# bramtoula/multi_robot_SLAM_separators

Hardware: AMD Instinct MI355X
Metric: candidate keyframe-pair verifications/sec (NetVLAD NN + ORB match + RANSAC) @1/2/4/8 GPU (higher is better)
Workload: dtype u8+f16+f32+f64

## Files before the change

### multi_robot_slam_separators_amd/csrc/k_match.hip

```cpp
#include "sf_internal.hpp"
#include <type_traits>

namespace {

__device__ __forceinline__ uint32_t bcnt_acc(uint32_t x, uint32_t acc) {
  uint32_t r;
  asm("v_bcnt_u32_b32 %0, %1, %2" : "=v"(r) : "v"(x), "v"(acc));
  return r;
}

template <int W, int NQ>
__device__ __forceinline__ void knn2_scan(const uint32_t* __restrict__ dF, int Kf, const uint32_t (&q)[NQ][W],
                                          uint32_t (&k1)[NQ], uint32_t (&k2)[NQ]) {
#pragma unroll 4
  for (int f = 0; f < Kf; ++f) {
    const uint32_t* r = dF + (size_t)f * W;
    uint32_t x[W];
#pragma unroll
    for (int c = 0; c < W; ++c) x[c] = r[c];
#pragma unroll
    for (int j = 0; j < NQ; ++j) {
      uint32_t d = 0;
#pragma unroll
      for (int c = 0; c < W; ++c) d = bcnt_acc(x[c] ^ q[j][c], d);
      const uint32_t key = (d << 16) | (uint32_t)f;
      k2[j] = min(max(key, k1[j]), k2[j]);
      k1[j] = min(k1[j], key);
    }
  }
}

template <int W>
__device__ __forceinline__ void knn2_scan_l2(const uint32_t* __restrict__ dF, int Kf, const uint32_t (&q)[W], float& d1,
                                             float& d2, int& i1) {
#pragma unroll 1
  for (int f = 0; f < Kf; ++f) {
    const uint32_t* r = dF + (size_t)f * W;
    float s = 0.f;
#pragma unroll
    for (int c = 0; c < W; ++c) {
      const float d = __uint_as_float(q[c]) - __uint_as_float(r[c]);
      s = s + d * d;
    }
    if (s < d1) { d2 = d1; d1 = s; i1 = f; }
    else if (s < d2) { d2 = s; }
  }
}

template <int W>
__device__ __forceinline__ void knn2_scan_l2_halves(const uint32_t* __restrict__ dF, int Kf,
                                                    const uint32_t* __restrict__ qrow, float& d1, float& d2, int& i1) {
  static_assert(W == 128, "two halves of 64 dimensions");
  constexpr int H = 64, FB = 16;
#pragma unroll 1
  for (int f0 = 0; f0 < Kf; f0 += FB) {
    float s[FB];
#pragma unroll
    for (int j = 0; j < FB; ++j) s[j] = 0.f;
#pragma unroll 1
    for (int half = 0; half < 2; ++half) {
      uint32_t q[H];
      {
        const uint4* p = reinterpret_cast<const uint4*>(qrow + half * H);
#pragma unroll
        for (int c = 0; c < H / 4; ++c) {
          const uint4 v = p[c];
          q[4 * c] = v.x; q[4 * c + 1] = v.y; q[4 * c + 2] = v.z; q[4 * c + 3] = v.w;
        }
      }
#pragma unroll
      for (int j = 0; j < FB; ++j) {
        if (f0 + j < Kf) {
          const uint32_t* r = dF + (size_t)(f0 + j) * W + half * H;
          float a = s[j];
#pragma unroll
          for (int c = 0; c < H; ++c) {
            const float d = __uint_as_float(q[c]) - __uint_as_float(r[c]);
            a = a + d * d;
          }
          s[j] = a;
        }
      }
    }
#pragma unroll
    for (int j = 0; j < FB; ++j) {
      if (f0 + j < Kf) {
        if (s[j] < d1) { d2 = d1; d1 = s[j]; i1 = f0 + j; }
        else if (s[j] < d2) { d2 = s[j]; }
      }
    }
  }
}

template <int W>
__device__ __forceinline__ void load_desc(const uint32_t* __restrict__ base, int row, bool valid, uint32_t (&q)[W]) {
  const uint4* p = reinterpret_cast<const uint4*>(base + (size_t)(valid ? row : 0) * W);
#pragma unroll
  for (int c = 0; c < W / 4; ++c) {
    uint4 v = p[c];
    q[4 * c + 0] = v.x; q[4 * c + 1] = v.y; q[4 * c + 2] = v.z; q[4 * c + 3] = v.w;
  }
}

template <int W, int NQ, int NT, bool L2 = false>
__global__ void __launch_bounds__(NT)
k_match_global(StoreView st, const int32_t* __restrict__ pair_from, const int32_t* __restrict__ pair_to,
               float nndr, int min_inliers, int est, uint32_t* __restrict__ corr, CorrHeader* __restrict__ hdr,
               PassState* __restrict__ pass, int32_t* __restrict__ list, int32_t* __restrict__ counter) {
  extern __shared__ __attribute__((aligned(16))) int smem[];
  constexpr int NW = NT / 64;
  const int pair = blockIdx.x;
  const int tid = threadIdx.x;
  const int lane = tid & 63, wave = tid >> 6;
  const int kcap = st.kcap;
  const int sF = pair_from[pair], sT = pair_to[pair];
  if ((unsigned)sF >= (unsigned)st.n_slots || (unsigned)sT >= (unsigned)st.n_slots) {
    if (tid == 0) {
      CorrHeader h = {0, 0, 0, 0};
      hdr[pair] = h;
      PassState ps;
#pragma unroll
      for (int i = 0; i < 12; ++i) ps.T[i] = 0.f;
      ps.var = 1.0; ps.var_ang = 1.0; ps.is_null = 1; ps.inliers = 0; ps.matches = 0; ps.pad = 0;
      pass[pair] = ps;
    }
    return;
  }
  const int4 mF = st.meta[sF], mT = st.meta[sT];
  const int Kf = mF.x, Kt = mT.x;
  const uint32_t* dF = st.desc + (size_t)sF * kcap * W;
  const uint32_t* dT = st.desc + (size_t)sT * kcap * W;

  int* cnt = smem;
  int* owner = smem + kcap;
  int* misc = smem + 2 * kcap;

  for (int i = tid; i < Kf; i += NT) cnt[i] = 0;
  if (tid < 16) misc[tid] = 0;
  __syncthreads();

  int rejected = 0;
  if constexpr (L2) {
    static_assert(!L2 || NQ == 1, "one resident float row per lane");
    if (Kf > 0) {
      for (int base = 0; base < Kt; base += NT) {
        const int t = base + tid;
        float d1 = __int_as_float(0x7F800000), d2 = __int_as_float(0x7F800000);
        int i1 = -1;
        if constexpr (W > 64) {
          if (Kt - base - (tid & ~63) > 0)
            knn2_scan_l2_halves<W>(dF, Kf, dT + (size_t)(t < Kt ? t : 0) * W, d1, d2, i1);
        } else {
          uint32_t q[W];
          load_desc<W>(dT, t, t < Kt, q);
          if (Kt - base - (tid & ~63) > 0)
            knn2_scan_l2<W>(dF, Kf, q, d1, d2, i1);
        }
        if (t < Kt) {
          const bool acc = (Kf >= 2) && i1 >= 0 && !(d1 > nndr * d2);
          if (acc) {
            atomicAdd(&cnt[i1], 1);
            owner[i1] = t;
          } else {
            ++rejected;
          }
        }
      }
    }
  } else
  if (Kf > 0) {
    for (int base = 0; base < Kt; base += NQ * NT) {
      uint32_t q[NQ][W], k1[NQ], k2[NQ];
#pragma unroll
      for (int j = 0; j < NQ; ++j) {
        const int t = base + j * NT + tid;
        load_desc<W>(dT, t, t < Kt, q[j]);
        k1[j] = 0xFFFFFFFFu;
        k2[j] = 0xFFFFFFFFu;
      }
      const int wave_rows = Kt - base - (tid & ~63);
      const int groups = wave_rows <= 0 ? 0 : min(NQ, (wave_rows + NT - 1) / NT);
      if (groups == NQ) {
        knn2_scan<W, NQ>(dF, Kf, q, k1, k2);
      } else if (groups > 0) {
#pragma unroll
        for (int j = 0; j < NQ; ++j) {
          if (j < groups) {
            uint32_t qq[1][W], a1[1] = {0xFFFFFFFFu}, a2[1] = {0xFFFFFFFFu};
#pragma unroll
            for (int c = 0; c < W; ++c) qq[0][c] = q[j][c];
            knn2_scan<W, 1>(dF, Kf, qq, a1, a2);
            k1[j] = a1[0];
            k2[j] = a2[0];
          }
        }
      }
#pragma unroll
      for (int j = 0; j < NQ; ++j) {
        const int t = base + j * NT + tid;
        if (t < Kt) {
          const bool acc = (Kf >= 2) && !((float)(k1[j] >> 16) > nndr * (float)(k2[j] >> 16));
          if (acc) {
            const int f = (int)(k1[j] & 0xFFFFu);
            atomicAdd(&cnt[f], 1);
            owner[f] = t;
          } else {
            ++rejected;
          }
        }
      }
    }
  }
  for (int off = 32; off >= 1; off >>= 1) rejected += __shfl_xor(rejected, off);
  if (lane == 0 && rejected) atomicAdd(&misc[0], rejected);
  __syncthreads();

  uint32_t* out = corr + (size_t)pair * kcap;
  int running = 0;
  for (int base = 0; base < Kf; base += NT) {
    const int f = base + tid;
    const bool flag = (f < Kf) && (cnt[f] == 1);
    const unsigned long long bal = __ballot(flag);
    const int before = __popcll(bal & ((1ull << lane) - 1ull));
    if (lane == 0) misc[4 + wave] = __popcll(bal);
    __syncthreads();
    int woff = 0, total = 0;
#pragma unroll
    for (int w = 0; w < NW; ++w) {
      int c = misc[4 + w];
      if (w < wave) woff += c;
      total += c;
    }
    if (flag) out[running + woff + before] = (uint32_t)f | ((uint32_t)owner[f] << 16);
    running += total;
    __syncthreads();
  }
  const int n_corr = running;

  const int unique_to = (Kf > 0 && Kt > 0) ? misc[0] + n_corr : 0;
  const int words_from = (Kf > 0 && mF.y > 0) ? Kf : 0;
  const int words_to = (mT.y > 0) ? unique_to : 0;
  const bool motion = est == 0 ? (unique_to > 0 && words_from >= min_inliers && words_to >= min_inliers)
                    : est == 1 ? (unique_to > 0 && words_from >= min_inliers && unique_to >= min_inliers)
                               : (est == 3 && unique_to > 0 && ((words_from >= min_inliers && unique_to >= min_inliers) ||
                                                                (words_to >= min_inliers && Kf >= min_inliers)));
  const bool survivor = est == 3 ? (motion && n_corr > 0) : (motion && n_corr >= min_inliers && n_corr >= (est == 0 ? 3 : 4));
  if (motion && !survivor) {
    const float* xF = st.xyz + (size_t)sF * kcap * 3;
    const float* xT = st.xyz + (size_t)sT * kcap * 3;
    for (int i = tid; i < n_corr; i += NT) {
      uint32_t c = out[i];
      const float* a = xF + 3 * (c & 0xFFFFu);
      const float* b = xT + 3 * (c >> 16);
      bool ok = isfinite(a[0]) && isfinite(a[1]) && isfinite(a[2]);
      if (est == 0)
        ok = ok && isfinite(b[0]) && isfinite(b[1]) && isfinite(b[2]) && (a[0] != 0.f || a[1] != 0.f || a[2] != 0.f) &&
             (b[0] != 0.f || b[1] != 0.f || b[2] != 0.f);
      if (ok) atomicAdd(&misc[2], 1);
    }
    __syncthreads();
  }
  if (tid == 0) {
    CorrHeader h;
    h.n_corr = n_corr;
    h.words_from = words_from;
    h.words_to = words_to;
    h.words_to_2d = unique_to;
    hdr[pair] = h;
    PassState ps;
#pragma unroll
    for (int i = 0; i < 12; ++i) ps.T[i] = 0.f;
    ps.var = 1.0; ps.var_ang = 1.0;
    ps.is_null = 1;
    ps.inliers = 0;
    ps.matches = (motion && !survivor) ? misc[2] : 0;
    ps.pad = 0;
    pass[pair] = ps;
    if (survivor) {
      int pos = atomicAdd(counter, 1);
      list[pos] = pair;
    }
  }
}

__device__ __forceinline__ uint32_t min_u16(uint32_t a, uint32_t b) {
  uint32_t r;
  asm("v_min_u16 %0, %1, %2" : "=v"(r) : "v"(a), "v"(b));
  return r;
}
__device__ __forceinline__ uint32_t max_u16(uint32_t a, uint32_t b) {
  uint32_t r;
  asm("v_max_u16 %0, %1, %2" : "=v"(r) : "v"(a), "v"(b));
  return r;
}

constexpr int MATCH_CH = 16;

template <int W, int NQ>
__device__ __forceinline__ void knn2_step_lds(const uint32_t* fromD, int f, const uint32_t (&q)[NQ][W],
                                              uint32_t (&d1)[NQ], uint32_t (&d2)[NQ]) {
  const uint4* r = reinterpret_cast<const uint4*>(fromD + (size_t)f * W);
  uint32_t x[W];
#pragma unroll
  for (int c = 0; c < W / 4; ++c) {
    const uint4 v = r[c];
    x[4 * c] = v.x; x[4 * c + 1] = v.y; x[4 * c + 2] = v.z; x[4 * c + 3] = v.w;
  }
#pragma unroll
  for (int j = 0; j < NQ; ++j) {
    uint32_t d = 0;
#pragma unroll
    for (int c = 0; c < W; ++c) d = bcnt_acc(x[c] ^ q[j][c], d);
    d2[j] = min_u16(d2[j], max_u16(d, d1[j]));
    d1[j] = min_u16(d1[j], d);
  }
}

template <int W, int NQ>
__device__ __forceinline__ void knn2_scan_lds(const uint32_t* fromD, int Kf, const uint32_t (&q)[NQ][W],
                                              uint32_t (&d1)[NQ], uint32_t (&d2)[NQ], uint32_t (&chunk)[NQ]) {
  int c0 = 0;
  for (; c0 + MATCH_CH <= Kf; c0 += MATCH_CH) {
    uint32_t prev[NQ];
#pragma unroll
    for (int j = 0; j < NQ; ++j) prev[j] = d1[j];
#pragma unroll 4
    for (int u = 0; u < MATCH_CH; ++u) knn2_step_lds<W, NQ>(fromD, c0 + u, q, d1, d2);
#pragma unroll
    for (int j = 0; j < NQ; ++j) chunk[j] = ((d1[j] & 0xFFFFu) != (prev[j] & 0xFFFFu)) ? (uint32_t)c0 : chunk[j];
  }
  if (c0 < Kf) {
    uint32_t prev[NQ];
#pragma unroll
    for (int j = 0; j < NQ; ++j) prev[j] = d1[j];
    for (int f = c0; f < Kf; ++f) knn2_step_lds<W, NQ>(fromD, f, q, d1, d2);
#pragma unroll
    for (int j = 0; j < NQ; ++j) chunk[j] = ((d1[j] & 0xFFFFu) != (prev[j] & 0xFFFFu)) ? (uint32_t)c0 : chunk[j];
  }
}

typedef int mf_v8i __attribute__((ext_vector_type(8)));
typedef float mf_v16f __attribute__((ext_vector_type(16)));
constexpr float MF_FR = 1.f / 2048.f;
constexpr int MF_MAX_ROWS = 2048;

__device__ __forceinline__ mf_v8i fp4_spread_from(uint32_t x, uint32_t m88, uint32_t c22) {
  mf_v8i o = {0, 0, 0, 0, 0, 0, 0, 0};
  o[0] = (int)((x & m88) | c22);
  o[1] = (int)(x & 0x44444444u);
  o[2] = (int)(x & 0x22222222u);
  o[3] = (int)(x & 0x11111111u);
  return o;
}
__device__ __forceinline__ mf_v8i fp4_spread_to(uint32_t y, uint32_t m88, uint32_t c22) {
  mf_v8i o = {0, 0, 0, 0, 0, 0, 0, 0};
  const uint32_t n = ~y;
  o[0] = (int)((y & m88) | c22);
  o[1] = (int)(((n << 1) & m88) | c22);
  o[2] = (int)(((n << 2) & m88) | 0x44444444u);
  o[3] = (int)(((n << 3) & m88) | 0x66666666u);
  return o;
}

static inline size_t sf_match_lds_bytes(int kcap, int w) {
  const int behind = 2 * kcap + 16;
  return (size_t)(kcap * w + (behind > 32 * w ? behind : 32 * w)) * sizeof(int);
}

template <int KS>
__device__ __forceinline__ void load_raw(const uint32_t* p, uint32_t (&raw)[KS]) {
#pragma unroll
  for (int c = 0; c < KS / 4; ++c) {
    const uint4 v = reinterpret_cast<const uint4*>(p)[c];
    raw[4 * c] = v.x; raw[4 * c + 1] = v.y; raw[4 * c + 2] = v.z; raw[4 * c + 3] = v.w;
  }
}

__device__ __forceinline__ void top2_update16(const mf_v16f& v, float& b, float& s) {
  float t = __builtin_amdgcn_fmed3f(v[0], v[1], INFINITY);
  float x;
  asm("v_max3_f32 %[t], %[t], %[o2], %[o3]\n\t"
      "v_max3_f32 %[t], %[t], %[o4], %[o5]\n\t"
      "v_max3_f32 %[t], %[t], %[o6], %[o7]\n\t"
      "v_max3_f32 %[t], %[t], %[o8], %[o9]\n\t"
      "v_max3_f32 %[t], %[t], %[o10], %[o11]\n\t"
      "v_max3_f32 %[t], %[t], %[o12], %[o13]\n\t"
      "v_max_f32 %[t], %[t], %[o14]\n\t"
      "v_med3_f32 %[x], %[b], %[t], %[o15]\n\t"
      "v_max3_f32 %[b], %[b], %[t], %[o15]\n\t"
      "v_max_f32 %[s], %[s], %[x]"
      : [b] "+v"(b), [s] "+v"(s), [t] "+v"(t), [x] "=&v"(x)
      : [o2] "v"(v[2]), [o3] "v"(v[3]), [o4] "v"(v[4]), [o5] "v"(v[5]), [o6] "v"(v[6]), [o7] "v"(v[7]), [o8] "v"(v[8]),
        [o9] "v"(v[9]), [o10] "v"(v[10]), [o11] "v"(v[11]), [o12] "v"(v[12]), [o13] "v"(v[13]), [o14] "v"(v[14]),
        [o15] "v"(v[15]));
}

template <int W, int NTL, bool TAIL>
__device__ __forceinline__ void knn2_mfma_tile(const uint32_t* fromD, int Kf, int mt, int r, int h,
                                               const mf_v8i (&Bf)[NTL][W / 2], const float (&cin)[16],
                                               float (&b)[NTL], float (&s)[NTL], uint32_t m88, uint32_t c22,
                                               uint32_t (&raw)[W / 2], const uint32_t*& nxt) {
  constexpr int KS = W / 2;
  mf_v16f c0;
#pragma unroll
  for (int i = 0; i < 16; ++i) c0[i] = cin[i];
  if (TAIL) {
    const float lim = -(float)(Kf - mt * 32) * MF_FR;
#pragma unroll
    for (int i = 0; i < 16; ++i) c0[i] = c0[i] > lim ? c0[i] : -INFINITY;
  }
  mf_v8i Af[KS];
#pragma unroll
  for (int k = 0; k < KS; ++k) Af[k] = fp4_spread_from(raw[k], m88, c22);
  if (!TAIL) {
    nxt += 32 * W;
    load_raw<KS>(nxt, raw);
  }
#pragma unroll
  for (int j = 0; j < NTL; ++j) {
    b[j] += 32.f * MF_FR;
    s[j] += 32.f * MF_FR;
  }
#pragma unroll
  for (int j = 0; j < NTL; ++j) {
    mf_v16f acc = __builtin_amdgcn_mfma_scale_f32_32x32x64_f8f6f4(Af[0], Bf[j][0], c0, 4, 4, 0, 0, 0, 0);
#pragma unroll
    for (int k = 1; k < KS; ++k)
      acc = __builtin_amdgcn_mfma_scale_f32_32x32x64_f8f6f4(Af[k], Bf[j][k], acc, 4, 4, 0, 0, 0, 0);
    top2_update16(acc, b[j], s[j]);
  }
}

template <int W, int NTL>
struct MfB {
  mf_v8i Bf[NTL][W / 2];
  uint32_t psum;
};

template <int W, int NTL>
__device__ __forceinline__ void mf_load_b(const uint32_t* __restrict__ dT, int Kt, const int (&tile)[NTL], int lane,
                                          MfB<W, NTL>& B) {
  constexpr int KS = W / 2;
  const int r = lane & 31, h = lane >> 5;
  uint32_t m88, c22;
  asm volatile("v_mov_b32 %0, 0x88888888" : "=v"(m88));
  asm volatile("v_mov_b32 %0, 0x22222222" : "=v"(c22));
  uint32_t raw[NTL][KS];
#pragma unroll
  for (int j = 0; j < NTL; ++j) load_raw<KS>(dT + (size_t)min(tile[j] * 32 + r, Kt - 1) * W + KS * h, raw[j]);
  static_assert(NTL == 1 || 24 * W < 256, "a tile's popcount fits its byte");
  uint32_t pk = 0;
#pragma unroll
  for (int j = 0; j < NTL; ++j) {
    uint32_t p = 0;
#pragma unroll
    for (int k = 0; k < KS; ++k) {
      B.Bf[j][k] = fp4_spread_to(raw[j][k], m88, c22);
      p += __popc(raw[j][k] & 0x77777777u);
    }
    pk |= p << (8 * j);
  }
  B.psum = pk + __shfl_xor(pk, 32);
}

typedef int mf_v4i __attribute__((ext_vector_type(4)));

__device__ __forceinline__ void mf_pipe_half1(mf_v16f& acc, const mf_v4i& a0, const mf_v4i& a1, const mf_v4i& a2,
                                              const mf_v4i& a3, const mf_v4i& b0, const mf_v4i& b1, const mf_v16f& cin,
                                              const mf_v16f& old, float& b, float& s, float& t) {
  asm volatile(
      "s_nop 1\n\t"
      "v_mfma_f32_32x32x64_f8f6f4 %[acc], %[a0], %[b0], %[cin] cbsz:4 blgp:4\n\t"
      "v_add_f32 %[b], 0x3c800000, %[b]\n\t"
      "v_add_f32 %[s], 0x3c800000, %[s]\n\t"
      "s_nop 4\n\t"
      "v_max3_f32 %[t], %[o0], %[o1], %[o2]\n\t"
      "v_mfma_f32_32x32x64_f8f6f4 %[acc], %[a1], %[b1], %[acc] cbsz:4 blgp:4\n\t"
      "v_max3_f32 %[t], %[t], %[o3], %[o4]\n\t"
      "v_max3_f32 %[t], %[t], %[o5], %[o6]\n\t"
      "v_max3_f32 %[t], %[t], %[o7], %[o8]"
      : [acc] "=&v"(acc), [b] "+v"(b), [s] "+v"(s), [t] "=&v"(t)
      : [a0] "v"(a0), [a1] "v"(a1), "v"(a2), "v"(a3), [b0] "v"(b0), [b1] "v"(b1), [cin] "v"(cin), [o0] "v"(old[0]),
        [o1] "v"(old[1]), [o2] "v"(old[2]), [o3] "v"(old[3]), [o4] "v"(old[4]), [o5] "v"(old[5]), [o6] "v"(old[6]),
        [o7] "v"(old[7]), [o8] "v"(old[8]));
}
__device__ __forceinline__ void mf_pipe_half2(mf_v16f& acc, const mf_v4i& a2, const mf_v4i& a3, const mf_v4i& b2,
                                              const mf_v4i& b3, const mf_v16f& old, float& b, float& s, float& t) {
  float x;
  asm volatile(
      "v_mfma_f32_32x32x64_f8f6f4 %[acc], %[a2], %[b2], %[acc] cbsz:4 blgp:4\n\t"
      "v_max3_f32 %[t], %[t], %[o9], %[o10]\n\t"
      "v_max3_f32 %[t], %[t], %[o11], %[o12]\n\t"
      "v_max3_f32 %[t], %[t], %[o13], %[o14]\n\t"
      "v_mfma_f32_32x32x64_f8f6f4 %[acc], %[a3], %[b3], %[acc] cbsz:4 blgp:4\n\t"
      "v_med3_f32 %[x], %[b], %[t], %[o15]\n\t"
      "v_max3_f32 %[b], %[b], %[t], %[o15]\n\t"
      "v_max_f32 %[s], %[s], %[x]"
      : [acc] "+v"(acc), [b] "+v"(b), [s] "+v"(s), [t] "+v"(t), [x] "=&v"(x)
      : [a2] "v"(a2), [a3] "v"(a3), [b2] "v"(b2), [b3] "v"(b3), [o9] "v"(old[9]), [o10] "v"(old[10]), [o11] "v"(old[11]),
        [o12] "v"(old[12]), [o13] "v"(old[13]), [o14] "v"(old[14]), [o15] "v"(old[15]));
}
__device__ __forceinline__ void mf_pipe_drain(const mf_v16f& old, float& b, float& s) {
  float t, x;
  asm volatile(
      "s_nop 11\n\t"
      "v_add_f32 %[b], 0x3c800000, %[b]\n\t"
      "v_add_f32 %[s], 0x3c800000, %[s]\n\t"
      "v_max3_f32 %[t], %[o0], %[o1], %[o2]\n\t"
      "v_max3_f32 %[t], %[t], %[o3], %[o4]\n\t"
      "v_max3_f32 %[t], %[t], %[o5], %[o6]\n\t"
      "v_max3_f32 %[t], %[t], %[o7], %[o8]\n\t"
      "v_max3_f32 %[t], %[t], %[o9], %[o10]\n\t"
      "v_max3_f32 %[t], %[t], %[o11], %[o12]\n\t"
      "v_max3_f32 %[t], %[t], %[o13], %[o14]\n\t"
      "v_med3_f32 %[x], %[b], %[t], %[o15]\n\t"
      "v_max3_f32 %[b], %[b], %[t], %[o15]\n\t"
      "v_max_f32 %[s], %[s], %[x]"
      : [b] "+v"(b), [s] "+v"(s), [t] "=&v"(t), [x] "=&v"(x)
      : [o0] "v"(old[0]), [o1] "v"(old[1]), [o2] "v"(old[2]), [o3] "v"(old[3]), [o4] "v"(old[4]), [o5] "v"(old[5]),
        [o6] "v"(old[6]), [o7] "v"(old[7]), [o8] "v"(old[8]), [o9] "v"(old[9]), [o10] "v"(old[10]), [o11] "v"(old[11]),
        [o12] "v"(old[12]), [o13] "v"(old[13]), [o14] "v"(old[14]), [o15] "v"(old[15]));
}

template <int NTL>
__device__ __forceinline__ void mf_scan_tiles_pipe(const uint32_t* fromD, int n_full, int tail, const MfB<8, NTL>& B,
                                                   const float (&cin)[16], float (&b)[NTL], float (&s)[NTL],
                                                   uint32_t m88, uint32_t c22, uint32_t (&raw)[4],
                                                   const uint32_t*& nxt) {
  static_assert(NTL == 2 || NTL == 4, "tiles alternate between two accumulator tuples");
  mf_v4i B4[NTL][4];
#pragma unroll
  for (int j = 0; j < NTL; ++j) {
#pragma unroll
    for (int k = 0; k < 4; ++k) B4[j][k] = mf_v4i{B.Bf[j][k][0], B.Bf[j][k][1], B.Bf[j][k][2], B.Bf[j][k][3]};
  }
  mf_v16f c0, acc0, acc1;
#pragma unroll
  for (int i = 0; i < 16; ++i) { c0[i] = cin[i]; acc1[i] = -INFINITY; }
#pragma unroll 1
  for (int pass = 0; pass < 2; ++pass) {
    int n = n_full, step = 32 * 8;
    if (pass) {
      if (!tail) break;
      const float lim = -(float)tail * MF_FR;
#pragma unroll
      for (int i = 0; i < 16; ++i) c0[i] = c0[i] > lim ? c0[i] : -INFINITY;
      n = 1; step = 0;
    }
    for (int mt = 0; mt < n; ++mt) {
      mf_v4i A4[4];
#pragma unroll
      for (int k = 0; k < 4; ++k) {
        const mf_v8i a = fp4_spread_from(raw[k], m88, c22);
        A4[k] = mf_v4i{a[0], a[1], a[2], a[3]};
      }
      nxt += step;
      load_raw<4>(nxt, raw);
#pragma unroll
      for (int j = 0; j < NTL; j += 2) {
        constexpr int JP = NTL - 1;
        float t;
        const int jp = j == 0 ? JP : j - 1;
        mf_pipe_half1(acc0, A4[0], A4[1], A4[2], A4[3], B4[j][0], B4[j][1], c0, acc1, b[jp], s[jp], t);
        mf_pipe_half2(acc0, A4[2], A4[3], B4[j][2], B4[j][3], acc1, b[jp], s[jp], t);
        mf_pipe_half1(acc1, A4[0], A4[1], A4[2], A4[3], B4[j + 1][0], B4[j + 1][1], c0, acc0, b[j], s[j], t);
        mf_pipe_half2(acc1, A4[2], A4[3], B4[j + 1][2], B4[j + 1][3], acc0, b[j], s[j], t);
      }
    }
  }
  mf_pipe_drain(acc1, b[NTL - 1], s[NTL - 1]);
}

__device__ __forceinline__ float mf_max(float a, float b) {
  float r;
  asm("v_max_f32 %0, %1, %2" : "=v"(r) : "v"(a), "v"(b));
  return r;
}
__device__ __forceinline__ float mf_min(float a, float b) {
  float r;
  asm("v_min_f32 %0, %1, %2" : "=v"(r) : "v"(a), "v"(b));
  return r;
}
__device__ __forceinline__ float mf_max3(float a, float b, float c) {
  float r;
  asm("v_max3_f32 %0, %1, %2, %3" : "=v"(r) : "v"(a), "v"(b), "v"(c));
  return r;
}

constexpr int mf_passes(int ntl) { return ntl == 1 ? 1 : ntl / 2; }

template <int W, int NTL, bool PIPE = false>
__device__ __forceinline__ void mf_scan(const uint32_t* fromD, int Kf, const MfB<W, NTL>& B, int lane,
                                        uint32_t (&d1)[mf_passes(NTL)], uint32_t (&d2)[mf_passes(NTL)],
                                        int (&idx)[mf_passes(NTL)]) {
  constexpr int KS = W / 2;
  const int r = lane & 31, h = lane >> 5;
  uint32_t m88, c22;
  asm volatile("v_mov_b32 %0, 0x88888888" : "=v"(m88));
  asm volatile("v_mov_b32 %0, 0x22222222" : "=v"(c22));
  float cin[16], b[NTL], s[NTL];
  const float hoff = h ? 4.f * MF_FR : 0.f;
#pragma unroll
  for (int i = 0; i < 16; ++i) cin[i] = -(float)((i & 3) + 8 * (i >> 2)) * MF_FR - hoff;
#pragma unroll
  for (int j = 0; j < NTL; ++j) { b[j] = -INFINITY; s[j] = -INFINITY; }
  const int n_full = Kf >> 5;
  uint32_t raw[KS];
  load_raw<KS>(fromD + (size_t)min(r, Kf - 1) * W + KS * h, raw);
  const uint32_t* nxt = fromD + (size_t)r * W + KS * h;
  if constexpr (PIPE && W == 8 && (NTL == 2 || NTL == 4)) {
    mf_scan_tiles_pipe<NTL>(fromD, n_full, Kf & 31, B, cin, b, s, m88, c22, raw, nxt);
  } else {
    for (int mt = 0; mt < n_full; ++mt) knn2_mfma_tile<W, NTL, false>(fromD, Kf, mt, r, h, B.Bf, cin, b, s, m88, c22, raw, nxt);
    if (Kf & 31) knn2_mfma_tile<W, NTL, true>(fromD, Kf, n_full, r, h, B.Bf, cin, b, s, m88, c22, raw, nxt);
  }
  const float org = (float)(32 * (((Kf + 31) >> 5) - 1)) * MF_FR;
#pragma unroll
  for (int p = 0; p < mf_passes(NTL); ++p) {
    float mb, ms, ob, os;
    int ts;
    if constexpr (NTL == 1) {
      mb = b[0]; ms = s[0]; ts = 24 * W - 2 * (int)B.psum;
      ob = __shfl_xor(mb, 32); os = __shfl_xor(ms, 32);
    } else {
      const int j0 = 2 * p, j1 = 2 * p + 1;
      mb = h ? b[j1] : b[j0]; ms = h ? s[j1] : s[j0]; ts = 24 * W - 2 * (int)((B.psum >> (16 * p + 8 * h)) & 0xFFu);
      ob = __shfl_xor(h ? b[j0] : b[j1], 32); os = __shfl_xor(h ? s[j0] : s[j1], 32);
    }
    const float nb = mf_max(mb, ob) - org;
    const float ns = mf_max3(mf_min(mb, ob), ms, os) - org;
    const float dot1 = 2.f * ceilf(nb * 0.5f), dot2 = 2.f * ceilf(ns * 0.5f);
    idx[p] = (int)((dot1 - nb) * 2048.f);
    d1[p] = (uint32_t)((32 * W - ts - (int)dot1) >> 1);
    d2[p] = ns == -INFINITY ? 0xFFFFu : (uint32_t)((32 * W - ts - (int)dot2) >> 1);
  }
}

template <int W, int NTL, bool PIPE = false>
__device__ __forceinline__ void knn2_mfma(const uint32_t* fromD, int Kf, const uint32_t* __restrict__ dT, int Kt,
                                          const int (&tile)[NTL], int lane, uint32_t (&d1)[mf_passes(NTL)],
                                          uint32_t (&d2)[mf_passes(NTL)], int (&idx)[mf_passes(NTL)]) {
  asm volatile("" : "+v"(lane));
  MfB<W, NTL> B;
  mf_load_b<W, NTL>(dT, Kt, tile, lane, B);
  mf_scan<W, NTL, PIPE>(fromD, Kf, B, lane, d1, d2, idx);
}

template <int W>
__device__ __forceinline__ uint32_t mf_repair_d2(const uint32_t* fromD, int Kf, const uint32_t* __restrict__ q_row, int idx,
                                                 uint32_t d2) {
  if ((idx & 27) == 27) return d2;
  uint32_t q[W];
  load_raw<W>(q_row, q);
  const int base = (idx & ~31) + (idx & 4);
#pragma unroll 1
  for (int g = 0; g < 32; g += 8) {
#pragma unroll
    for (int k = 0; k < 4; ++k) {
      const int row = base + g + k;
      uint32_t x[W];
      load_raw<W>(fromD + (size_t)row * W, x);
      uint32_t d = 0;
#pragma unroll
      for (int c = 0; c < W; ++c) d = bcnt_acc(x[c] ^ q[c], d);
      const bool other = row < Kf && row != idx && (g + k) != 27;
      d2 = other ? min(d2, d) : d2;
    }
  }
  return d2;
}

template <int W, int NQ, int NT, int MF_NTL = 2, bool MF_PIPE = false>
__device__ __forceinline__ bool match_v2_body(const StoreView& st, int pair, int sF, int sT, float nndr, int min_inliers,
                                              int est, uint32_t* out, CorrHeader& hdr_out, PassState& pass_out,
                                              int32_t* __restrict__ list, int32_t* __restrict__ counter, int* smem,
                                              unsigned long long* trace_row = nullptr) {
  constexpr int NW = NT / 64;
  const int tid = threadIdx.x;
  const int lane = tid & 63, wave = __builtin_amdgcn_readfirstlane(tid >> 6);
  const int kcap = st.kcap;
  if ((unsigned)sF >= (unsigned)st.n_slots || (unsigned)sT >= (unsigned)st.n_slots) {
    if (tid == 0) {
      CorrHeader h = {0, 0, 0, 0};
      hdr_out = h;
      PassState ps;
#pragma unroll
      for (int i = 0; i < 12; ++i) ps.T[i] = 0.f;
      ps.var = 1.0; ps.var_ang = 1.0; ps.is_null = 1; ps.inliers = 0; ps.matches = 0; ps.pad = 0;
      pass_out = ps;
    }
    return false;
  }
  const int4 mF = st.meta[sF], mT = st.meta[sT];
  const int Kf = mF.x, Kt = mT.x;
  const uint32_t* dF = st.desc + (size_t)sF * kcap * W;
  const uint32_t* dT = st.desc + (size_t)sT * kcap * W;

  uint32_t* fromD = reinterpret_cast<uint32_t*>(smem);
  int* cnt = smem + kcap * W;
  int* owner = cnt + kcap;
  int* misc = owner + kcap;

  {
    const uint4* src = reinterpret_cast<const uint4*>(dF);
    uint4* dst = reinterpret_cast<uint4*>(fromD);
    for (int i = tid; i < Kf * (W / 4); i += NT) dst[i] = src[i];
  }
  for (int i = tid; i < Kf; i += NT) cnt[i] = 0;
  if (tid < 16) misc[tid] = 0;
  __syncthreads();
  SF_TRACE_ROW_MARK(trace_row, 32);

  int rejected = 0;
  if constexpr (NQ == 0) {
    if (Kf > 0) {
      constexpr int NTL = W == 8 ? MF_NTL : 1;
      const int n_nt = (Kt + 31) >> 5;
      auto group = [&](auto g, int t0) {
        constexpr int G = decltype(g)::value, NP = mf_passes(G);
        int tl[G], f[NP];
        uint32_t a1[NP], a2[NP];
#pragma unroll
        for (int j = 0; j < G; ++j) tl[j] = t0 + j * NW;
        knn2_mfma<W, G, MF_PIPE>(fromD, Kf, dT, Kt, tl, lane, a1, a2, f);
#pragma unroll
        for (int p = 0; p < NP; ++p) {
          const int t = G == 1 ? tl[0] * 32 + lane : (tl[2 * p] + (lane >> 5) * NW) * 32 + (lane & 31);
          const bool on = (G > 1 || lane < 32) && t < Kt;
          bool acc = (Kf >= 2) && !((float)a1[p] > nndr * (float)a2[p]);
          const bool redo = on && Kf >= 2 && (acc || nndr < 0.f);
          if (__ballot(redo)) {
            if (redo) {
              a2[p] = mf_repair_d2<W>(fromD, Kf, dT + (size_t)t * W, f[p], a2[p]);
              acc = !((float)a1[p] > nndr * (float)a2[p]);
            }
          }
          if (on && acc) {
            atomicAdd(&cnt[f[p]], 1);
            owner[f[p]] = t;
          }
          rejected += __popcll(__ballot(on && !acc));
        }
      };
      for (int t0 = wave; t0 < n_nt; t0 += NW * NTL) {
        const int avail = (n_nt - t0 + NW - 1) / NW;
        if constexpr (NTL >= 4) {
          if (avail >= 3) { group(std::integral_constant<int, 4>{}, t0); continue; }
        }
        if constexpr (NTL >= 2) {
          if (avail >= 2) { group(std::integral_constant<int, 2>{}, t0); continue; }
        }
        group(std::integral_constant<int, 1>{}, t0);
      }
    }
  } else if (Kf > 0) {
    for (int base = 0; base < Kt; base += NQ * NT) {

      uint32_t q[NQ][W], d1[NQ], d2[NQ], chunk[NQ];
#pragma unroll
      for (int j = 0; j < NQ; ++j) {
        const int t = base + j * NT + tid;
        load_desc<W>(dT, t, t < Kt, q[j]);
        d1[j] = 0xFFFFu;
        d2[j] = 0xFFFFu;
        chunk[j] = 0;
      }
      const int wave_rows = Kt - base - (tid & ~63);
      const int groups = wave_rows <= 0 ? 0 : min(NQ, (wave_rows + NT - 1) / NT);
      if (groups == NQ) {
        knn2_scan_lds<W, NQ>(fromD, Kf, q, d1, d2, chunk);
      } else if (groups > 0) {
#pragma unroll
        for (int j = 0; j < NQ; ++j) {
          if (j < groups) {
            uint32_t qq[1][W], a1[1] = {0xFFFFu}, a2[1] = {0xFFFFu}, ch[1] = {0};
#pragma unroll
            for (int c = 0; c < W; ++c) qq[0][c] = q[j][c];
            knn2_scan_lds<W, 1>(fromD, Kf, qq, a1, a2, ch);
            d1[j] = a1[0]; d2[j] = a2[0]; chunk[j] = ch[0];
          }
        }
      }
#pragma unroll
      for (int j = 0; j < NQ; ++j) {
        const int t = base + j * NT + tid;
        if (t < Kt) {
          const uint32_t b1 = d1[j] & 0xFFFFu, b2 = d2[j] & 0xFFFFu;
          const bool acc = (Kf >= 2) && !((float)b1 > nndr * (float)b2);
          if (acc) {
            int f = (int)chunk[j];
            const int fend = min(f + MATCH_CH, Kf);
            for (; f < fend; ++f) {
              const uint32_t* r = fromD + (size_t)f * W;
              uint32_t d = 0;
#pragma unroll
              for (int c = 0; c < W; ++c) d += __popc(r[c] ^ q[j][c]);
              if (d == b1) break;
            }
            atomicAdd(&cnt[f], 1);
            owner[f] = t;
          } else {
            ++rejected;
          }
        }
      }
    }
  }
  if constexpr (NQ != 0) {
    for (int off = 32; off >= 1; off >>= 1) rejected += __shfl_xor(rejected, off);
  }
  if (lane == 0 && rejected) atomicAdd(&misc[0], rejected);
  SF_TRACE_ROW_MARK(trace_row, 33);
  __syncthreads();
  SF_TRACE_ROW_MARK(trace_row, 34);

  int running = 0;
  for (int base = 0; base < Kf; base += NT) {
    const int f = base + tid;
    const bool flag = (f < Kf) && (cnt[f] == 1);
    const unsigned long long bal = __ballot(flag);
    const int before = __popcll(bal & ((1ull << lane) - 1ull));
    if (lane == 0) misc[4 + wave] = __popcll(bal);
    __syncthreads();
    int woff = 0, total = 0;
#pragma unroll
    for (int w = 0; w < NW; ++w) {
      int c = misc[4 + w];
      if (w < wave) woff += c;
      total += c;
    }
    if (flag) out[running + woff + before] = (uint32_t)f | ((uint32_t)owner[f] << 16);
    running += total;
    __syncthreads();
  }
  const int n_corr = running;
  SF_TRACE_ROW_MARK(trace_row, 35);

  const int unique_to = (Kf > 0 && Kt > 0) ? misc[0] + n_corr : 0;
  const int words_from = (Kf > 0 && mF.y > 0) ? Kf : 0;
  const int words_to = (mT.y > 0) ? unique_to : 0;
  const bool motion = est == 0 ? (unique_to > 0 && words_from >= min_inliers && words_to >= min_inliers)
                    : est == 1 ? (unique_to > 0 && words_from >= min_inliers && unique_to >= min_inliers)
                               : (est == 3 && unique_to > 0 && ((words_from >= min_inliers && unique_to >= min_inliers) ||
                                                                (words_to >= min_inliers && Kf >= min_inliers)));
  const bool survivor = est == 3 ? (motion && n_corr > 0) : (motion && n_corr >= min_inliers && n_corr >= (est == 0 ? 3 : 4));
  if (motion && !survivor) {
    const float* xF = st.xyz + (size_t)sF * kcap * 3;
    const float* xT = st.xyz + (size_t)sT * kcap * 3;
    for (int i = tid; i < n_corr; i += NT) {
      uint32_t c = out[i];
      const float* a = xF + 3 * (c & 0xFFFFu);
      const float* b = xT + 3 * (c >> 16);
      bool ok = isfinite(a[0]) && isfinite(a[1]) && isfinite(a[2]);
      if (est == 0)
        ok = ok && isfinite(b[0]) && isfinite(b[1]) && isfinite(b[2]) && (a[0] != 0.f || a[1] != 0.f || a[2] != 0.f) &&
             (b[0] != 0.f || b[1] != 0.f || b[2] != 0.f);
      if (ok) atomicAdd(&misc[2], 1);
    }
    __syncthreads();
  }
  if (tid == 0) {
    CorrHeader h;
    h.n_corr = n_corr;
    h.words_from = words_from;
    h.words_to = words_to;
    h.words_to_2d = unique_to;
    hdr_out = h;
    PassState ps;
#pragma unroll
    for (int i = 0; i < 12; ++i) ps.T[i] = 0.f;
    ps.var = 1.0; ps.var_ang = 1.0;
    ps.is_null = 1;
    ps.inliers = 0;
    ps.matches = (motion && !survivor) ? misc[2] : 0;
    ps.pad = 0;
    pass_out = ps;
    if (survivor && list) {
      int pos = atomicAdd(counter, 1);
      list[pos] = pair;
    }
  }
  return survivor;
}

template <int W, int NQ, int NT>
__global__ void __launch_bounds__(NT)
k_match_global_v2(StoreView st, const int32_t* __restrict__ pair_from, const int32_t* __restrict__ pair_to,
                  float nndr, int min_inliers, int est, uint32_t* __restrict__ corr, CorrHeader* __restrict__ hdr,
                  PassState* __restrict__ pass, int32_t* __restrict__ list, int32_t* __restrict__ counter) {
  extern __shared__ __attribute__((aligned(16))) int smem[];
  const int pair = (int)blockIdx.x;
  match_v2_body<W, NQ, NT>(st, pair, pair_from[pair], pair_to[pair], nndr, min_inliers, est, corr + (size_t)pair * st.kcap,
                           hdr[pair], pass[pair], list, counter, smem);
}

template <int W, int NT>
__global__ void __launch_bounds__(NT, 2)
k_match_global_mf(StoreView st, const int32_t* __restrict__ pair_from, const int32_t* __restrict__ pair_to,
                  float nndr, int min_inliers, int est, uint32_t* __restrict__ corr, CorrHeader* __restrict__ hdr,
                  PassState* __restrict__ pass, int32_t* __restrict__ list, int32_t* __restrict__ counter) {
  extern __shared__ __attribute__((aligned(16))) int smem[];
  const int pair = (int)blockIdx.x;
  match_v2_body<W, 0, NT, 4>(st, pair, pair_from[pair], pair_to[pair], nndr, min_inliers, est,
                             corr + (size_t)pair * st.kcap, hdr[pair], pass[pair], list, counter, smem);
}

template <int W, int NQ, int NT>
void launch_match_v2(sf_context* c, StoreView st, const int32_t* d_from, const int32_t* d_to, int n) {
  size_t lds = sf_match_lds_bytes(st.kcap, W);
  if (const char* v = getenv("SF_MATCH_LDS_PAD")) lds += (size_t)atoi(v);
  int32_t* counters = (int32_t*)c->w->counters.p;
  if constexpr (NQ == 0)
    hipLaunchKernelGGL((k_match_global_mf<W, NT>), dim3(n), dim3(NT), lds, c->stream, st, d_from, d_to,
                       c->dparams.nndr, c->dparams.min_inliers, sf_est_mode(c), (uint32_t*)c->w->corr1.p,
                       (CorrHeader*)c->w->hdr1.p, (PassState*)c->w->pass1.p, (int32_t*)c->w->list1.p, counters + 0);
  else
    hipLaunchKernelGGL((k_match_global_v2<W, NQ, NT>), dim3(n), dim3(NT), lds, c->stream, st, d_from, d_to,
                       c->dparams.nndr, c->dparams.min_inliers, sf_est_mode(c), (uint32_t*)c->w->corr1.p,
                       (CorrHeader*)c->w->hdr1.p, (PassState*)c->w->pass1.p, (int32_t*)c->w->list1.p, counters + 0);
}

template <int W, int NQ, int NT>
void launch_match(sf_context* c, StoreView st, const int32_t* d_from, const int32_t* d_to, int n) {
  const size_t lds = (size_t)(2 * st.kcap + 16) * sizeof(int);
  int32_t* counters = (int32_t*)c->w->counters.p;
  hipLaunchKernelGGL((k_match_global<W, NQ, NT>), dim3(n), dim3(NT), lds, c->stream, st, d_from, d_to,
                     c->dparams.nndr, c->dparams.min_inliers, sf_est_mode(c), (uint32_t*)c->w->corr1.p, (CorrHeader*)c->w->hdr1.p,
                     (PassState*)c->w->pass1.p, (int32_t*)c->w->list1.p, counters + 0);
}

template <int W>
void launch_match_l2(sf_context* c, StoreView st, const int32_t* d_from, const int32_t* d_to, int n) {
  const size_t lds = (size_t)(2 * st.kcap + 16) * sizeof(int);
  int32_t* counters = (int32_t*)c->w->counters.p;
  hipLaunchKernelGGL((k_match_global<W, 1, 256, true>), dim3(n), dim3(256), lds, c->stream, st, d_from, d_to,
                     c->dparams.nndr, c->dparams.min_inliers, sf_est_mode(c), (uint32_t*)c->w->corr1.p, (CorrHeader*)c->w->hdr1.p,
                     (PassState*)c->w->pass1.p, (int32_t*)c->w->list1.p, counters + 0);
}

}

int sf_launch_match_global(sf_context* c, StoreView st, const int32_t* d_from, const int32_t* d_to, int n) {
  if (n <= 0) return SF_OK;
  if (c->params.desc_type == 1) {
    sf_prof_begin(c, SF_K_MATCH);
    if (st.w == 64) launch_match_l2<64>(c, st, d_from, d_to, n);
    else launch_match_l2<128>(c, st, d_from, d_to, n);
    sf_prof_end(c, SF_K_MATCH);
    SF_HIP(c, hipGetLastError());
    return SF_OK;
  }
  int variant = c->match_variant;
  if (variant == 0) {
    const size_t lds_v2 = sf_match_lds_bytes(st.kcap, st.w);
    variant = lds_v2 <= 64 * 1024 ? (c->match_mfma && st.kcap <= MF_MAX_ROWS ? 10256 : 12256) : 2256;
  }
  sf_prof_begin(c, SF_K_MATCH);
#define SF_CASE(NQ_, NT_)                                                        \
  case NQ_ * 1000 + NT_:                                                         \
    if (st.w == 8) launch_match<8, NQ_, NT_>(c, st, d_from, d_to, n);            \
    else launch_match<16, NQ_, NT_>(c, st, d_from, d_to, n);                     \
    break;
  switch (variant) {
    SF_CASE(1, 256)
    SF_CASE(2, 256)
    SF_CASE(4, 128)
    SF_CASE(2, 128)
    SF_CASE(4, 256)
    SF_CASE(8, 64)
    SF_CASE(4, 64)
#define SF_CASE2(NQ_, NT_)                                                          \
  case 10000 + NQ_ * 1000 + NT_:                                                    \
    if (st.w == 8) launch_match_v2<8, NQ_, NT_>(c, st, d_from, d_to, n);            \
    else launch_match_v2<16, NQ_, NT_>(c, st, d_from, d_to, n);                     \
    break;
    SF_CASE2(0, 256)
    SF_CASE2(2, 256)
    SF_CASE2(1, 256)
    SF_CASE2(4, 128)
    SF_CASE2(2, 128)
#undef SF_CASE2
    default:
      sf_prof_end(c, SF_K_MATCH);
      return sf_fail(c, SF_EINVAL, "unknown match kernel variant %d", variant);
  }
#undef SF_CASE
  sf_prof_end(c, SF_K_MATCH);
  SF_HIP(c, hipGetLastError());
  return SF_OK;
}
```

Baseline: 26.41 million.

## Compact NNDR repair lanes across passes and add cheap early-accept repair check

Adds a fast repair path that scans only the ambiguous 32-row block with a 4-word partial popcount. It accepts early when even the lower-bound second distance passes the ratio test, and falls back to the exact mf_repair_d2 otherwise. For two-pass groups, lanes needing repair from both passes are packed into one wavefront with ds_permute/bpermute, so only one repair iteration runs instead of two divergent ones. It also rewrites the FP4 spread for the B operand with SGPR/VGPR constants to trim ALU ops. The costs are extra permute traffic and more complex logic whose correctness depends on the bit-mask bookkeeping and 16-bit packing of t/f/a1/a2.

```diff
diff --git a/multi_robot_slam_separators_amd/csrc/k_match.hip b/multi_robot_slam_separators_amd/csrc/k_match.hip
--- a/multi_robot_slam_separators_amd/csrc/k_match.hip
+++ b/multi_robot_slam_separators_amd/csrc/k_match.hip
@@ -352,13 +352,16 @@
   o[3] = (int)(x & 0x11111111u);
   return o;
 }
-__device__ __forceinline__ mf_v8i fp4_spread_to(uint32_t y, uint32_t m88, uint32_t c22) {
+struct FpB {
+  uint32_t c2, c4, c6;
+  uint32_t e2, e4, e6;
+};
+__device__ __forceinline__ mf_v8i fp4_spread_to(uint32_t y, uint32_t m88, uint32_t c22, const FpB& K) {
   mf_v8i o = {0, 0, 0, 0, 0, 0, 0, 0};
-  const uint32_t n = ~y;
   o[0] = (int)((y & m88) | c22);
-  o[1] = (int)(((n << 1) & m88) | c22);
-  o[2] = (int)(((n << 2) & m88) | 0x44444444u);
-  o[3] = (int)(((n << 3) & m88) | 0x66666666u);
+  o[1] = (int)(K.e2 ^ ((y << 1) & (K.c2 ^ K.e2)));
+  o[2] = (int)(K.e4 ^ ((y << 2) & (K.c4 ^ K.e4)));
+  o[3] = (int)(K.e6 ^ ((y << 3) & (K.c6 ^ K.e6)));
   return o;
 }
 
@@ -445,6 +448,13 @@
   uint32_t m88, c22;
   asm volatile("v_mov_b32 %0, 0x88888888" : "=v"(m88));
   asm volatile("v_mov_b32 %0, 0x22222222" : "=v"(c22));
+  FpB K;
+  asm volatile("s_mov_b32 %0, 0x22222222" : "=s"(K.c2));
+  asm volatile("s_mov_b32 %0, 0x44444444" : "=s"(K.c4));
+  asm volatile("s_mov_b32 %0, 0x66666666" : "=s"(K.c6));
+  asm volatile("v_mov_b32 %0, 0xaaaaaaaa" : "=v"(K.e2));
+  asm volatile("v_mov_b32 %0, 0xcccccccc" : "=v"(K.e4));
+  asm volatile("v_mov_b32 %0, 0xeeeeeeee" : "=v"(K.e6));
   uint32_t raw[NTL][KS];
 #pragma unroll
   for (int j = 0; j < NTL; ++j) load_raw<KS>(dT + (size_t)min(tile[j] * 32 + r, Kt - 1) * W + KS * h, raw[j]);
@@ -455,7 +465,7 @@
     uint32_t p = 0;
 #pragma unroll
     for (int k = 0; k < KS; ++k) {
-      B.Bf[j][k] = fp4_spread_to(raw[j][k], m88, c22);
+      B.Bf[j][k] = fp4_spread_to(raw[j][k], m88, c22, K);
       p += __popc(raw[j][k] & 0x77777777u);
     }
     pk |= p << (8 * j);
@@ -670,6 +680,47 @@
   return d2;
 }
 
+__device__ __forceinline__ int mf_rank_below(unsigned long long mask) {
+  return (int)__builtin_amdgcn_mbcnt_hi((uint32_t)(mask >> 32), __builtin_amdgcn_mbcnt_lo((uint32_t)mask, 0u));
+}
+
+template <int W>
+__device__ __forceinline__ bool mf_repair_accept(const uint32_t* fromD, int Kf, const uint32_t* __restrict__ q_row, int idx,
+                                                 uint32_t d1, uint32_t d2, float nndr, bool active) {
+  bool acc = false, exact = active;
+  if (nndr >= 0.f) {
+    if (active) {
+      uint32_t pmin = d2;
+      if ((idx & 27) != 27) {
+        uint32_t q[4];
+        load_raw<4>(q_row, q);
+        const int base = (idx & ~31) + (idx & 4);
+        const uint32_t ok = ((1u << min(Kf - base, 31)) - 1u) & ~(1u << (idx - base)) & ~(1u << 27);
+        uint32_t no = __builtin_amdgcn_alignbit(~ok, ~ok, 23);
+#pragma unroll 1
+        for (int g = 0; g < 32; g += 8) {
+#pragma unroll
+          for (int k = 0; k < 4; ++k) {
+            uint32_t x[4];
+            load_raw<4>(fromD + (size_t)(base + g + k) * W, x);
+            uint32_t p = no & (512u << k);
+#pragma unroll
+            for (int c = 0; c < 4; ++c) p = bcnt_acc(x[c] ^ q[c], p);
+            pmin = min(pmin, p);
+          }
+          no = __builtin_amdgcn_alignbit(no, no, 8);
+        }
+      }
+      acc = !((float)d1 > nndr * (float)pmin);
+      exact = !acc;
+    }
+  }
+  if (__ballot(exact)) {
+    if (exact) acc = !((float)d1 > nndr * (float)mf_repair_d2<W>(fromD, Kf, q_row, idx, d2));
+  }
+  return acc;
+}
+
 template <int W, int NQ, int NT, int MF_NTL = 2, bool MF_PIPE = false>
 __device__ __forceinline__ bool match_v2_body(const StoreView& st, int pair, int sF, int sT, float nndr, int min_inliers,
                                               int est, uint32_t* out, CorrHeader& hdr_out, PassState& pass_out,
@@ -723,23 +774,69 @@
 #pragma unroll
         for (int j = 0; j < G; ++j) tl[j] = t0 + j * NW;
         knn2_mfma<W, G, MF_PIPE>(fromD, Kf, dT, Kt, tl, lane, a1, a2, f);
+        int t[NP];
+        bool on[NP], acc[NP], redo[NP];
 #pragma unroll
         for (int p = 0; p < NP; ++p) {
-          const int t = G == 1 ? tl[0] * 32 + lane : (tl[2 * p] + (lane >> 5) * NW) * 32 + (lane & 31);
-          const bool on = (G > 1 || lane < 32) && t < Kt;
-          bool acc = (Kf >= 2) && !((float)a1[p] > nndr * (float)a2[p]);
-          const bool redo = on && Kf >= 2 && (acc || nndr < 0.f);
-          if (__ballot(redo)) {
-            if (redo) {
-              a2[p] = mf_repair_d2<W>(fromD, Kf, dT + (size_t)t * W, f[p], a2[p]);
-              acc = !((float)a1[p] > nndr * (float)a2[p]);
+          t[p] = G == 1 ? tl[0] * 32 + lane : (tl[2 * p] + (lane >> 5) * NW) * 32 + (lane & 31);
+          on[p] = (G > 1 || lane < 32) && t[p] < Kt;
+          acc[p] = (Kf >= 2) && !((float)a1[p] > nndr * (float)a2[p]);
+          redo[p] = on[p] && Kf >= 2 && (acc[p] || !(nndr >= 0.f));
+        }
+        if constexpr (NP == 1) {
+          if (__ballot(redo[0])) {
+            const bool r = mf_repair_accept<W>(fromD, Kf, dT + (size_t)t[0] * W, f[0], a1[0], a2[0], nndr, redo[0]);
+            acc[0] = redo[0] ? r : acc[0];
+          }
+        } else {
+          static_assert(NP == 2, "a group has one or two decode passes");
+          const unsigned long long bal0 = __ballot(redo[0]), bal1 = __ballot(redo[1]);
+          const int n0 = __popcll(bal0), n1 = __popcll(bal1);
+          const bool merged = nndr >= 0.f && n0 != 0 && n1 != 0 && n0 + n1 <= 64;
+          int tgt = 0;
+          uint32_t m0 = 0, m1 = 0;
+          bool mine = false;
+          if (merged) {
+            const int jf = mf_rank_below(~bal0), r1 = mf_rank_below(bal1);
+            const int dest = redo[0] ? 64 - n0 + lane - jf : jf;
+            const int slot = __builtin_amdgcn_ds_permute(dest << 2, lane);
+            tgt = __builtin_amdgcn_ds_bpermute((redo[1] ? r1 : n1 + lane - r1) << 2, slot);
+            m0 = (uint32_t)__builtin_amdgcn_ds_permute(tgt << 2, (int)((uint32_t)t[1] | ((uint32_t)f[1] << 16)));
+            m1 = (uint32_t)__builtin_amdgcn_ds_permute(tgt << 2, (int)(a1[1] | (a2[1] << 16)));
+            mine = !redo[0] && jf < n1;
+          }
+#pragma unroll 1
+          for (int it = 0; it < 2; ++it) {
+            bool act = it ? redo[1] : redo[0];
+            int wt = it ? t[1] : t[0], wf = it ? f[1] : f[0];
+            uint32_t w1 = it ? a1[1] : a1[0], w2 = it ? a2[1] : a2[0];
+            if (mine) {
+              act = true;
+              wt = (int)(m0 & 0xFFFFu); wf = (int)(m0 >> 16);
+              w1 = m1 & 0xFFFFu; w2 = m1 >> 16;
             }
+            if (__ballot(act)) {
+              const bool r = mf_repair_accept<W>(fromD, Kf, dT + (size_t)wt * W, wf, w1, w2, nndr, act);
+              if (merged) {
+                const bool back = __builtin_amdgcn_ds_bpermute(tgt << 2, (int)r) != 0;
+                acc[0] = redo[0] ? r : acc[0];
+                acc[1] = redo[1] ? back : acc[1];
+              } else if (it) {
+                acc[1] = redo[1] ? r : acc[1];
+              } else {
+                acc[0] = redo[0] ? r : acc[0];
+              }
+            }
+            if (merged) break;
           }
-          if (on && acc) {
+        }
+#pragma unroll
+        for (int p = 0; p < NP; ++p) {
+          if (on[p] && acc[p]) {
             atomicAdd(&cnt[f[p]], 1);
-            owner[f[p]] = t;
+            owner[f[p]] = t[p];
           }
-          rejected += __popcll(__ballot(on && !acc));
+          rejected += __popcll(__ballot(on[p] && !acc[p]));
         }
       };
       for (int t0 = wave; t0 < n_nt; t0 += NW * NTL) {
```

Result: faster. 26.76 million (median of 6 runs) (+1.3%).
